# DanMcGann/loam

Measured on AMD Instinct MI355X. Metric: scan-pair registrations/sec (64x1024 Ouster), higher is better.
Workload: dtype f64; 1 GPU; batch of 1024 independent 64x1024 scan pairs per GPU (BASELINE configs[2]/[3]); step = extractFeatures x2 + registerFeatures per pair, inputs resident in HBM; pairs_per_gpu=1024, scan=64x1024, seed=20240311, input_scalar=f64, arithmetic=f64 (float input is widened on load)

## Files before the change

include/loamx.h:

```cpp
#ifndef LOAMX_H_
#define LOAMX_H_

#include <stddef.h>
#include <stdint.h>

#ifdef __cplusplus
extern "C" {
#endif

typedef struct loamx_ctx loamx_ctx;

enum {
  LOAMX_OK = 0,
  LOAMX_ERR_SCAN_SIZE = 1,
  LOAMX_ERR_BAD_PARAM = 2,
  LOAMX_ERR_HIP = 3,
  LOAMX_ERR_CAPACITY = 4,
  LOAMX_ERR_UNSUPPORTED = 5,
  LOAMX_ERR_NO_DEVICE = 6,
  LOAMX_ERR_COMM = 7
};

typedef struct {
  uint64_t scan_lines;
// ... 91 lines not shown
enum {
  LOAMX_WALK_NONE = 0,
  LOAMX_WALK_FLAT = 1,
  LOAMX_WALK_TILED_BY_COUNT = 2,
  LOAMX_WALK_TILED_BY_TILES = 3
};
typedef struct {
  uint32_t iterations, termination;
  uint32_t use_moments;
  uint32_t mom_ref_on;
  double mom_ref[7];
  uint32_t tiles;
  uint32_t live_tiles;
  uint64_t edge_stride, planar_stride;
  uint32_t n_se, n_sp;
  uint32_t walk;
  uint32_t listed_total;
  double s0max, v2max;
  uint32_t sweep_chunk, edge_cache, list_cache, flat_cache;
  uint32_t* tile_counts;
  size_t tile_counts_cap;
} loamx_solve_census;
int loamx_ctx_last_solve_census(loamx_ctx* ctx, size_t pair, loamx_solve_census* out);
enum { LOAMX_ASSOC_SEARCH_NONE = 0, LOAMX_ASSOC_SEARCH_BRUTE = 1, LOAMX_ASSOC_SEARCH_GRID = 2 };
enum { LOAMX_ASSOC_LEFTOVER_NONE = 0, LOAMX_ASSOC_LEFTOVER_LEFT = 1, LOAMX_ASSOC_LEFTOVER_COOP = 2 };
#define LOAMX_ASSOC_REASON_WIDE 0x80000000u
#define LOAMX_ASSOC_REASON_TIED 0x40000000u
typedef struct {
  uint32_t n_src, n_tgt;
  uint64_t stride;
  uint32_t km;
  uint32_t search;
  uint32_t mixed_launch;
  uint32_t one_stage;
  uint32_t leftover_kernel;
  uint32_t rest_blocks, coop_blocks;
  uint32_t rest_spread, left_spread;
  uint32_t lean_set;
  double origin[3], h;
  int32_t nx, ny, nz;
  uint32_t n_points;
  uint32_t verified, unverified, queued_words;
  uint32_t queued, queued_plain, queued_wide, queued_tied;
  uint32_t rest_searched;
  uint32_t listed;
  uint32_t leftover_finished;
// ... 525 lines not shown
```

loam_amd/capi.py:

```python
import collections
import ctypes as C
import os

import numpy as np

from . import build as _build

OK, ERR_SCAN_SIZE, ERR_BAD_PARAM, ERR_HIP, ERR_CAPACITY, ERR_UNSUPPORTED, ERR_NO_DEVICE, ERR_COMM = range(8)
CONVERGED, MAX_ITER, INSUFFICIENT_ASSOCIATIONS = 0, 1, 2
K_CURVATURE, K_SELECT, K_COMPACT, K_GRID, K_ASSOC, K_SWEEP, K_LM, K_MOMENT, K_KNN_PLANE, K_EXTRACT_FUSED, K_INFORMATION, K_CLOUD_ACCUMULATE, K_CLOUD_ACCUMULATE_PLAIN, K_CLOUD_LIST, K_CLOUD_EMIT, K_COUNT = range(16)


class LidarParams(C.Structure):
    _fields_ = [("scan_lines", C.c_uint64), ("points_per_line", C.c_uint64), ("min_range", C.c_double),
                ("max_range", C.c_double)]


class FeatureExtractionParams(C.Structure):
    _fields_ = [("neighbor_points", C.c_uint64), ("number_sectors", C.c_uint64),
                ("max_edge_feats_per_sector", C.c_uint64), ("max_planar_feats_per_sector", C.c_uint64),
                ("edge_feat_threshold", C.c_double), ("planar_feat_threshold", C.c_double),
                ("occlusion_thresh", C.c_double), ("parallel_thresh", C.c_double)]

    def __init__(self, *a, **kw):
# ... 317 lines not shown
PGO_LINEARIZATION_DTYPE = np.dtype([("e", np.float64, 6), ("chi2", np.float64), ("weight", np.float64), ("A", np.float64, (6, 6)),
                                    ("B", np.float64, (6, 6))])
PGO_TERMINATIONS = ("COST_CONVERGED", "STEP_CONVERGED", "MAX_ITERATIONS", "LAMBDA_OVERFLOW", "NOTHING_TO_DO", "BAD_INPUT")
(PGO_COST_CONVERGED, PGO_STEP_CONVERGED, PGO_MAX_ITERATIONS, PGO_LAMBDA_OVERFLOW, PGO_NOTHING_TO_DO, PGO_BAD_INPUT) = range(6)


EXPORTS = [
    "loamx_default_fe_params", "loamx_default_reg_params", "loamx_status_string", "loamx_last_error",
    "loamx_ctx_create", "loamx_ctx_destroy", "loamx_ctx_set_stream", "loamx_ctx_synchronize",
    "loamx_compute_curvature", "loamx_compute_valid_points", "loamx_extract_features", "loamx_register_features",
    "loamx_target_index_create", "loamx_target_index_destroy", "loamx_register_features_indexed",
    "loamx_edge_capacity", "loamx_planar_capacity", "loamx_extract_features_batch_dev",
    "loamx_register_features_batch_dev", "loamx_register_scan_pairs_dev", "loamx_register_scan_pairs",
    "loamx_register_scan_pairs_f32", "loamx_ctx_enable_kernel_timing",
    "loamx_ctx_reset_kernel_stats", "loamx_ctx_get_kernel_stats", "loamx_kernel_name", "loamx_synth_pair_pose",
    "loamx_synth_scan_host", "loamx_synth_scan_pairs_dev", "loamx_dev_alloc", "loamx_dev_free",
    "loamx_copy_to_device", "loamx_copy_to_host",
    "loamx_compute_curvature_f32", "loamx_compute_valid_points_f32", "loamx_extract_features_f32",
    "loamx_extract_features_batch_dev_f32", "loamx_register_scan_pairs_dev_f32",
    "loamx_target_index_insert", "loamx_target_index_size", "loamx_target_index_census",
    "loamx_shard_range", "loamx_comm_get_unique_id", "loamx_comm_create", "loamx_comm_wrap", "loamx_comm_destroy",
    "loamx_comm_info", "loamx_gather_results_dev", "loamx_comm_barrier", "loamx_comm_stats", "loamx_ctx_extract_counters",
    "loamx_ctx_set_option", "loamx_ctx_get_option", "loamx_ctx_last_extract_route", "loamx_ctx_last_solve_census",
    "loamx_ctx_last_assoc_census",
    "loamx_ctx_last_assoc_coop_forms",
    "loamx_fit_lines", "loamx_fit_planes", "loamx_knn_search", "loamx_associate", "loamx_target_index_stats",
    "loamx_register_scan_sequence_dev", "loamx_register_scan_sequence_dev_f32", "loamx_register_scan_sequence",
    "loamx_register_scan_sequence_f32", "loamx_compose_trajectory_dev", "loamx_deskew_scans_dev", "loamx_deskew_scans_dev_f32",
    "loamx_deskew_launch_geometry",
    "loamx_target_index_points", "loamx_voxel_filter_dev", "loamx_target_index_insert_filtered", "loamx_target_index_crop",
    "loamx_registration_information", "loamx_registration_information_indexed", "loamx_registration_information_batch_dev",
    "loamx_register_scan_pairs_info_dev", "loamx_register_scan_pairs_info_dev_f32", "loamx_register_scan_sequence_info_dev",
    "loamx_register_scan_sequence_info_dev_f32",
    "loamx_default_organize_params", "loamx_scan_layout_create", "loamx_scan_layout_destroy", "loamx_scan_layout_tables",
    "loamx_organize_clouds_dev", "loamx_organize_clouds_dev_f32", "loamx_organize_cloud", "loamx_organize_cloud_f32",
    "loamx_default_place_params", "loamx_place_db_create", "loamx_place_db_destroy", "loamx_place_db_sector_dirs", "loamx_place_db_size",
    "loamx_place_descriptors_dev", "loamx_place_descriptors_dev_f32", "loamx_place_db_add_dev", "loamx_place_db_read",
    "loamx_place_search_dev", "loamx_place_descriptor", "loamx_place_descriptor_f32", "loamx_place_search",
    "loamx_pgo_default_params", "loamx_pose_graph_optimize_dev", "loamx_pose_graph_optimize", "loamx_pose_graph_linearize",
    "loamx_pose_graph_edges_from_results_dev",
    "loamx_default_cloud_map_params", "loamx_cloud_map_create", "loamx_cloud_map_destroy", "loamx_cloud_map_clear",
    "loamx_cloud_map_add_clouds_dev", "loamx_cloud_map_add_clouds_dev_f32", "loamx_cloud_map_emit_dev", "loamx_cloud_map_stats_read",
    "loamx_cloud_map_add_cloud", "loamx_cloud_map_add_cloud_f32", "loamx_cloud_map_emit", "loamx_cloud_map_claims_read",
    "loamx_default_segment_params", "loamx_segment_constants", "loamx_segment_scans_dev", "loamx_segment_scans_dev_f32",
    "loamx_segment_scan", "loamx_segment_scan_f32", "loamx_ctx_last_segment_census",
    "loamx_default_visibility_params", "loamx_visibility_votes_dev", "loamx_visibility_votes_dev_f32", "loamx_visibility_filter_dev",
    "loamx_visibility_votes", "loamx_visibility_votes_f32", "loamx_ctx_last_visibility_census",
# ... 177 lines not shown
    lib.loamx_copy_to_host.argtypes = [vp, vp, vp, C.c_size_t]
    szp = C.POINTER(C.c_size_t)
    lib.loamx_shard_range.argtypes = [C.c_size_t, C.c_int, C.c_int, szp, szp]
    lib.loamx_shard_range.restype = None
    lib.loamx_comm_get_unique_id.argtypes = [C.c_char_p]
    lib.loamx_comm_create.argtypes = [vp, C.c_char_p, C.c_int, C.c_int, C.POINTER(vp)]
    lib.loamx_comm_wrap.argtypes = [vp, vp, C.POINTER(vp)]
    lib.loamx_comm_destroy.argtypes = [vp]
    lib.loamx_comm_destroy.restype = None
    lib.loamx_comm_info.argtypes = [vp, C.POINTER(C.c_int), C.POINTER(C.c_int), C.POINTER(C.c_int)]
    lib.loamx_gather_results_dev.argtypes = [vp, vp, vp, C.c_size_t, C.c_size_t, vp]
    lib.loamx_comm_barrier.argtypes = [vp, vp, dp]
    lib.loamx_comm_stats.argtypes = [vp, C.POINTER(C.c_uint64)]
    lib.loamx_ctx_extract_counters.argtypes = [vp, C.POINTER(C.c_uint64), C.POINTER(C.c_uint64)]
    lib.loamx_fit_lines.argtypes = [vp, dp, C.c_size_t, C.c_size_t, dp, dp]
    lib.loamx_fit_planes.argtypes = [vp, dp, C.c_size_t, C.c_size_t, dp, dp]
    lib.loamx_knn_search.argtypes = [vp, vp, C.c_int, dp, C.c_size_t, C.c_size_t, C.c_double, vp, vp]
    lib.loamx_associate.argtypes = [vp, dp, C.c_size_t, dp, C.c_size_t, dp, C.c_size_t, dp, C.c_size_t, dp,
                                    C.POINTER(RegistrationParams), C.POINTER(AssocDump)]
    lib.loamx_ctx_set_option.argtypes = [vp, C.c_char_p, C.c_int]
    lib.loamx_ctx_get_option.argtypes = [vp, C.c_char_p, C.POINTER(C.c_int)]
    lib.loamx_ctx_last_extract_route.argtypes = [vp, C.POINTER(C.c_uint32)]
    lib.loamx_ctx_last_solve_census.argtypes = [vp, C.c_size_t, C.POINTER(SolveCensusStruct)]
    lib.loamx_ctx_last_assoc_census.argtypes = [vp, C.c_int, C.POINTER(AssocCensusStruct)]
    lib.loamx_ctx_last_assoc_coop_forms.argtypes = [vp, C.c_int, u32p]
    lib.loamx_registration_information.argtypes = [vp, dp, C.c_size_t, dp, C.c_size_t, dp, C.c_size_t, dp, C.c_size_t, dp,
                                                   C.POINTER(RegistrationParams), C.POINTER(RegInformation)]
    lib.loamx_registration_information_indexed.argtypes = [vp, vp, dp, C.c_size_t, dp, C.c_size_t, dp, C.POINTER(RegistrationParams),
                                                           C.POINTER(RegInformation)]
    lib.loamx_registration_information_batch_dev.argtypes = lib.loamx_register_features_batch_dev.argtypes
    lib.loamx_register_scan_pairs_info_dev.argtypes = lib.loamx_register_scan_pairs_dev.argtypes + [vp]
    lib.loamx_register_scan_pairs_info_dev_f32.argtypes = lib.loamx_register_scan_pairs_info_dev.argtypes
    lib.loamx_register_scan_sequence_info_dev.argtypes = lib.loamx_register_scan_sequence_dev.argtypes + [vp]
    lib.loamx_register_scan_sequence_info_dev_f32.argtypes = lib.loamx_register_scan_sequence_info_dev.argtypes
    lib.loamx_default_organize_params.argtypes = [C.POINTER(OrganizeParamsStruct)]
    lib.loamx_default_organize_params.restype = None
    lib.loamx_scan_layout_create.argtypes = [vp, C.POINTER(LidarParams), C.POINTER(OrganizeParamsStruct), C.POINTER(vp)]
    lib.loamx_scan_layout_destroy.argtypes = [vp, vp]
    lib.loamx_scan_layout_destroy.restype = None
    lib.loamx_scan_layout_tables.argtypes = [vp, dp, dp]
    lib.loamx_organize_clouds_dev.argtypes = [vp, vp, vp, C.c_size_t, vp, szp, C.c_size_t, vp, vp, vp]
    lib.loamx_organize_clouds_dev_f32.argtypes = lib.loamx_organize_clouds_dev.argtypes
    lib.loamx_organize_cloud.argtypes = [vp, vp, vp, C.c_size_t, vp, C.c_size_t, vp, vp, vp]
    lib.loamx_organize_cloud_f32.argtypes = lib.loamx_organize_cloud.argtypes
    lib.loamx_default_place_params.argtypes = [C.POINTER(PlaceParamsStruct)]
    lib.loamx_default_place_params.restype = None
# ... 591 lines not shown
        self._check(self.lib.loamx_ctx_get_option(self.h, name.encode(), C.byref(v)))
        return v.value

    def extract_counters(self):
        a, b = C.c_uint64(0), C.c_uint64(0)
        self._check(self.lib.loamx_ctx_extract_counters(self.h, C.byref(a), C.byref(b)))
        return a.value, b.value

    def last_extract_route(self):
        v = C.c_uint32(0)
        self._check(self.lib.loamx_ctx_last_extract_route(self.h, C.byref(v)))
        return ExtractRoute(v.value)

    def last_solve_census(self, pair=0):
        v = SolveCensusStruct()
        self._check(self.lib.loamx_ctx_last_solve_census(self.h, pair, C.byref(v)))
        counts = np.zeros(max(1, v.live_tiles), dtype=np.uint32)
        v.tile_counts, v.tile_counts_cap = counts.ctypes.data_as(C.POINTER(C.c_uint32)), v.live_tiles
        self._check(self.lib.loamx_ctx_last_solve_census(self.h, pair, C.byref(v)))
        return SolveCensus(v.iterations, v.termination, v.use_moments, v.mom_ref_on, np.array(list(v.mom_ref)), v.tiles, v.live_tiles,
                           v.edge_stride, v.planar_stride, v.n_se, v.n_sp, v.walk, v.listed_total, v.s0max, v.v2max, v.sweep_chunk,
                           v.edge_cache, v.list_cache, v.flat_cache, counts[:v.live_tiles].copy())

    def last_assoc_coop_forms(self, kind):
        kind = {"edge": 0, "plane": 1}.get(kind, kind)
        out = (C.c_uint32 * 2)()
        self._check(self.lib.loamx_ctx_last_assoc_coop_forms(self.h, kind, out))
        return int(out[0]), int(out[1])

    def last_assoc_census(self, kind):
        kind = {"edge": 0, "plane": 1}.get(kind, kind)
        v = AssocCensusStruct()
        self._check(self.lib.loamx_ctx_last_assoc_census(self.h, kind, C.byref(v)))
        q = int(v.queued)
        eq, er = np.zeros(max(1, q), dtype=np.uint32), np.zeros(max(1, q), dtype=np.uint32)
        ar, bf = np.zeros(max(1, q), dtype=np.int32), np.zeros(max(1, q), dtype=np.int32)
        v.entry_query, v.entry_reason = eq.ctypes.data_as(C.POINTER(C.c_uint32)), er.ctypes.data_as(C.POINTER(C.c_uint32))
        v.count_after_rest, v.count_before_fit = ar.ctypes.data_as(C.POINTER(C.c_int32)), bf.ctypes.data_as(C.POINTER(C.c_int32))
        v.entries_cap = q
        nl = int(v.late)
        lq = np.zeros(max(1, nl), dtype=np.uint32)
        v.late_query, v.late_cap = lq.ctypes.data_as(C.POINTER(C.c_uint32)), nl
        self._check(self.lib.loamx_ctx_last_assoc_census(self.h, kind, C.byref(v)))
        return AssocCensus(*[getattr(v, n) for n in ASSOC_CENSUS_SCALARS], np.array(list(v.origin)), eq[:q].copy(), er[:q].copy(),
                           ar[:q].copy(), bf[:q].copy(), lq[:nl].copy())

# ... 537 lines not shown
```

loam_amd/csrc/api_core.hip:

```cpp
#include "api_host.h"
#include "synth.h"

using namespace loamx;

namespace loamx {
thread_local LaunchScope* g_launch_scope = nullptr;
int g_debug_sync = getenv("LOAMX_DEBUG_SYNC") ? 1 : 0;
thread_local uint32_t g_extract_route = 0;
}

namespace {

const char* kKernelNames[LOAMX_K_COUNT] = {"curvature_valid_kernel", "select_kernel", "compact_kernel",
                                           "grid_build_kernel",      "associate_kernel", "sweep_kernel",
                                           "lm_kernels",             "moment_kernel",    "knn_plane_kernel",
                                           "extract_fused_kernel",   "information_kernel", "cloud_accumulate_kernel",
                                           "cloud_accumulate_plain_kernel", "cloud_list_kernels", "cloud_emit_kernels"};

struct OptionName {
  const char* name;
  bool extract;
  uint32_t bit;
};
const OptionName kOptionNames[] = {
    {"FORCE_TIE_REPLAY", true, kFlagForceReplay}, {"FORCE_SCAN_GIVEUP", true, kFlagForceGiveUp}, {"CURV_V1", true, kFlagCurvV1},
    {"NO_FUSED_COMPACT", true, kFlagNoFusedCompact}, {"NO_MIS_SELECT", true, kFlagNoMisSelect}, {"FUSED_EXTRACT", true, kFlagFusedExtract},
    {"NO_ROW_SELECT", true, kFlagNoRowSelect}, {"FUSED_ROWS", true, kFlagFusedRows}, {"NO_SPLIT_CURV", true, kFlagNoSplitCurv}, {"STAGE_ALWAYS", true, kFlagStageAlways},
    {"NO_MOMENTS", false, kRegFlagNoMoments}, {"NO_PACKED_GRID", false, kRegFlagNoPackedGrid}, {"NO_BIG_GRID", false, kRegFlagNoBigGrid},
    {"NO_GRID_SIDE", false, kRegFlagNoGridSide}, {"DEBUG_POISON", false, kRegFlagPoison},
    {"QUEUE_TWO_STAGE", false, kRegFlagQueueTwoStage}, {"QUEUE_ONE_STAGE", false, kRegFlagQueueOneStage},
    {"NO_MIXED_ASSOC", false, kRegFlagNoMixedAssoc}, {"FORCE_RCCL", false, kRegFlagForceRccl},
    {"NO_COOP_LEFT", false, kRegFlagNoCoopLeft}, {"NO_COOP_ROWS", false, kRegFlagNoCoopRows}, {"NO_REF_MOMENTS", false, kRegFlagNoRefMoments},
    {"NO_EXTRACT_BOXES", false, kRegFlagNoExtractBoxes}, {"CHECK_FINITE", false, kRegFlagCheckFinite},
    {"NO_SMALL_SETS", false, kRegFlagNoSmallSets}, {"FORCE_LATE_VERIFY", false, kRegFlagForceLate},
    {"NO_LIVE_DEAL", false, kRegFlagNoLiveDeal}, {"NO_CLOUDMAP_COMBINE", false, kRegFlagNoCloudmapCombine},
    {"NO_SEGMENT_TILES", false, kRegFlagNoSegmentTiles}, {"NO_VISIBILITY_RANGES", false, kRegFlagNoVisibilityRanges},
    {"NO_OCCUPANCY_COMBINE", false, kRegFlagNoOccupancyCombine}};

}

namespace loamx {

int fail(loamx_ctx* ctx, int code, const std::string& msg) {
  if (ctx) ctx->last_error = msg;
  return code;
}

int ensure(loamx_ctx* ctx, Buf& b, size_t bytes) {
  if (bytes == 0) bytes = 8;
  if (b.cap >= bytes) return LOAMX_OK;
  if (b.p) {
    HIP_TRY(ctx, hipStreamSynchronize(ctx->stream));
    HIP_TRY(ctx, hipFree(b.p));
    b.p = nullptr, b.cap = 0;
  }
  HIP_TRY(ctx, hipMalloc(&b.p, bytes));
  b.cap = bytes;
  return LOAMX_OK;
}
int ensure(loamx_ctx* ctx, int id, size_t bytes) { return ensure(ctx, ctx->ws[id], bytes); }
// ... 424 lines not shown
```

loam_amd/csrc/api_register.hip:

```cpp
#include "api_host.h"

using namespace loamx;

namespace {

int enqueue_association(loamx_ctx* ctx, const RegBatch& B, const RegConfig& C, uint32_t what = kAssocEdges | kAssocPlanes,
                        AssocCensusRun* census = nullptr) {
  hipStream_t s = ctx->stream;
  {
    TimedScope t(ctx, LOAMX_K_ASSOC, 0.0);
    const bool side = (size_t)B.n_pairs * B.kind[kPlane].assoc_blocks >= 128;
    PendingEvent knn{};
    LaunchScope knn_ls{nullptr, nullptr, true};
    if (ctx->timing) {
      knn.kernel = LOAMX_K_KNN_PLANE, knn.bytes = 0.0, knn.own_e0 = true;
      knn.e0 = take_event(ctx), knn.e1 = take_event(ctx);
      knn_ls = LaunchScope{knn.e0, knn.e1, true};
    }
    launch_associate(B, C, s, side ? ctx->aux_stream : nullptr, side ? ctx->aux2_stream : nullptr, ctx->ev_fork, ctx->ev_mid, ctx->ev_join,
                     ctx->ev_join2, ctx->timing ? &knn_ls : nullptr, what, census);
    if (ctx->timing) {
      if (knn_ls.first) ctx->event_pool.push_back(knn.e0), ctx->event_pool.push_back(knn.e1);
      else ctx->pending.push_back(knn);
    }
// ... 11 lines not shown
#ifdef LOAMX_NN_SAME_STATS
  debug_nn_same(B, it, s);
#endif
  if (hook) {
    untimed(ctx);
    int rc = hook(ctx, B, it, hook_user);
    if (rc != LOAMX_OK) return rc;
  }
  {
    TimedScope t(ctx, LOAMX_K_LM, 0.0, true);
    launch_lm_begin(B, C, s);
  }
  const bool ref_first = it == 0 && B.ref_moments != 0u;
  if (ref_first) {
    {
      TimedScope t(ctx, LOAMX_K_SWEEP, 0.0, true);
      launch_sweep(B, s);
    }
    TimedScope t(ctx, LOAMX_K_LM, 0.0, true);
    launch_lm_step(B, s);
  }
  if (it > 0 || ref_first) {
    TimedScope t(ctx, LOAMX_K_MOMENT, 0.0, true);
    launch_moments(B, s);
  }
  if (it > 0 || ref_first) {
    TimedScope t(ctx, LOAMX_K_LM, 0.0, true);
    launch_lm_pair_loop(B, C, s);
  } else {
    for (int k = 0; k < 5; k++) {
      {
        TimedScope t(ctx, LOAMX_K_SWEEP, 0.0, true);
        launch_sweep(B, s);
      }
      {
        TimedScope t(ctx, LOAMX_K_LM, 0.0, true);
        launch_lm_step(B, s);
      }
    }
  }
  CHECK_LAUNCH(ctx, "sweep/lm kernels");
  if (it == 0 && !ref_first) {
    TimedScope t(ctx, LOAMX_K_LM, 0.0, true);
    launch_outer_update(B, C, s);
  }
  CHECK_LAUNCH(ctx, "outer_update_kernel");
  return LOAMX_OK;
// ... 456 lines not shown
  out->tiles = B.mom_blocks_per_pair * 4;
  out->edge_stride = B.kind[kEdge].stride, out->planar_stride = B.kind[kPlane].stride;
  out->n_se = n_raw[kEdge] < B.kind[kEdge].stride ? n_raw[kEdge] : (uint32_t)B.kind[kEdge].stride;
  out->n_sp = n_raw[kPlane] < B.kind[kPlane].stride ? n_raw[kPlane] : (uint32_t)B.kind[kPlane].stride;
  out->sweep_chunk = (uint32_t)kSweepChunk, out->edge_cache = kEdgeCache, out->list_cache = kListCache, out->flat_cache = kFlatCache;
  uint32_t live = 0;
  while (live < out->tiles && (size_t)(live / 4) * kSweepChunk < out->n_sp) live++;
  out->live_tiles = live;
  const bool lists = !(ctx->last_solve_flags & kRegFlagNoMoments) && (S.iterations >= 2u || S.mom_ref_on != 0u);
  if (!lists) return LOAMX_OK;
  double maxima[2];
  HIP_TRY(ctx, hipMemcpy(maxima, B.moments + pair * (size_t)(kMomSize + 2) + kMomSize, sizeof(maxima), hipMemcpyDeviceToHost));
  out->s0max = maxima[0], out->v2max = maxima[1];
  std::vector<uint32_t> cnt(live);
  if (live) HIP_TRY(ctx, hipMemcpy(cnt.data(), B.flagged_count + pair * (size_t)out->tiles, live * sizeof(uint32_t), hipMemcpyDeviceToHost));
  for (uint32_t t = 0; t < live; t++) {
    out->listed_total += cnt[t];
    if (t < cap) counts_out[t] = cnt[t];
  }
  out->walk = out->tiles > kListCache ? LOAMX_WALK_TILED_BY_TILES : (out->listed_total > kFlatCache ? LOAMX_WALK_TILED_BY_COUNT : LOAMX_WALK_FLAT);
  return LOAMX_OK;
}

int loamx_ctx_last_assoc_census(loamx_ctx* ctx, int which_kind, loamx_assoc_census* out) {
  if (!out) return LOAMX_ERR_BAD_PARAM;
  API_LOCK(ctx);
  if (which_kind != 0 && which_kind != 1) return fail(ctx, LOAMX_ERR_BAD_PARAM, "which_kind: 0 = edges, 1 = planes");
  if (!ctx->last_assoc_census_valid) return fail(ctx, LOAMX_ERR_BAD_PARAM, "no association dump on this context to read (or another call came after it)");
  const loamx_ctx::AssocCensusKept& keep = ctx->last_assoc_census[which_kind];
  uint32_t *const eq = out->entry_query, *const er = out->entry_reason;
  int32_t *const ar = out->count_after_rest, *const bf = out->count_before_fit;
  const size_t cap = out->entries_cap, lcap = out->late_cap;
  uint32_t* const lq = out->late_query;
  *out = keep.c;
  out->late_query = lq, out->late_cap = lcap;
  for (size_t t = 0; lq && t < keep.late.size() && t < lcap; t++) lq[t] = keep.late[t];
  out->entry_query = eq, out->entry_reason = er, out->count_after_rest = ar, out->count_before_fit = bf, out->entries_cap = cap;
  for (size_t t = 0; t < keep.entry.size() && t < cap; t++) {
    if (eq) eq[t] = keep.entry[t] & 0x3FFFFFFFu;
    if (er) er[t] = keep.entry[t] & (LOAMX_ASSOC_REASON_WIDE | LOAMX_ASSOC_REASON_TIED);
    if (ar) ar[t] = keep.after_rest[t];
    if (bf) bf[t] = keep.before_fit[t];
  }
  return LOAMX_OK;
}

// ... 146 lines not shown
```

loam_amd/csrc/loamx_internal.h:

```cpp
#pragma once
#include <hip/hip_runtime.h>
#include <hip/hip_ext.h>
#include <stdint.h>
#include <stdio.h>

#include <vector>

#include "../../include/loamx.h"
#include "extract_math.h"
#include "reg_math.h"
#include "organize_math.h"
#include "place_math.h"
#include "segment_math.h"
#include "visibility_math.h"
#include "occupancy_math.h"
#include "xcd_map.h"

namespace loamx {

struct LaunchScope {
  hipEvent_t start, stop;
  bool first;
};
extern thread_local LaunchScope* g_launch_scope;
// ... 85 lines not shown
  RegKindConfig kind[2];
  double min_line_cond, max_avg_plane_dist;
  uint32_t max_iterations;
  double rot_thresh, pos_thresh;
  uint32_t min_associations;
  uint32_t flags;
};
constexpr uint32_t kRegFlagNoMoments = 1u;
constexpr uint32_t kRegFlagNoPackedGrid = 2u;
constexpr uint32_t kRegFlagNoBigGrid = 4u;
constexpr uint32_t kRegFlagNoGridSide = 8u;
constexpr uint32_t kRegFlagPoison = 16u;
constexpr uint32_t kRegFlagQueueTwoStage = 32u;
constexpr uint32_t kRegFlagQueueOneStage = 64u;
constexpr uint32_t kRegFlagForceRccl = 256u;
constexpr uint32_t kRegFlagNoCoopLeft = 512u;
constexpr uint32_t kRegFlagNoCoopRows = 131072u;
constexpr uint32_t kRegFlagNoRefMoments = 1024u;
constexpr uint32_t kRegFlagNoSmallSets = 8192u;
constexpr uint32_t kRegFlagCheckFinite = 4096u;
constexpr uint32_t kRegFlagNoExtractBoxes = 2048u;
constexpr uint32_t kRegFlagNoMixedAssoc = 128u;
constexpr uint32_t kRegFlagNoLiveDeal = 32768u;
constexpr uint32_t kRegFlagForceLate = 16384u;

struct GridSet {
  GridDesc* desc;
  uint32_t* cell_start;
  GridPoint* sorted;
  size_t stride;
  float* rel;
  uint32_t cells_cap;
};

struct RegKind {
  size_t stride;
  const double* src;
  const uint32_t* n_src;
  const double* tgt;
  const uint32_t* n_tgt;
  GridSet grid;
  GridSet src_grid;
  uint32_t knn_mode;
  uint32_t assoc_blocks;
  double* rec;
  uint32_t* nn;
// ... 95 lines not shown
};
struct AssocCensusBuf {
  uint32_t* counts;
  int32_t* after_rest;
  int32_t* before_fit;
};
struct AssocCensusRun {
  AssocCensusForm form[2];
  AssocCensusBuf buf[2];
};
void assoc_census_derive(const AssocCensusForm& F, size_t n_pairs, const GridDesc& g, const uint32_t* rest, uint32_t queued, uint32_t listed,
                         uint32_t out[4]);
constexpr uint32_t kAssocEdges = 1u, kAssocPlanes = 2u;
void launch_associate(const RegBatch& B, const RegConfig& C, hipStream_t s, hipStream_t aux, hipStream_t aux2, hipEvent_t ev_fork,
                      hipEvent_t ev_mid, hipEvent_t ev_join, hipEvent_t ev_join2, LaunchScope* knn_scope = nullptr,
                      uint32_t what = kAssocEdges | kAssocPlanes, AssocCensusRun* census = nullptr);
#ifdef LOAMX_NN_SAME_STATS
void debug_nn_same(const RegBatch& B, uint32_t it, hipStream_t s);
#endif
void launch_lm_begin(const RegBatch& B, const RegConfig& C, hipStream_t s);
void launch_sweep(const RegBatch& B, hipStream_t s);
void launch_lm_pair_loop(const RegBatch& B, const RegConfig& C, hipStream_t s);
void launch_lm_step(const RegBatch& B, hipStream_t s);
void launch_moments(const RegBatch& B, hipStream_t s);
void launch_outer_update(const RegBatch& B, const RegConfig& C, hipStream_t s);
void launch_write_results(const RegBatch& B, loamx_reg_result* d_results, hipStream_t s);

size_t index_insert_ws_bytes(size_t cells, size_t n_add);
void launch_index_insert_count(const GridSet& gs, size_t cells, const double* d_add, uint32_t n_add, void* ws, hipStream_t s);
void launch_index_insert_merge(const GridSet& gs, size_t cells, uint32_t n_old, const double* d_add, uint32_t n_add, void* ws,
                               GridPoint* sorted2, float* rel2, hipStream_t s);

constexpr int kFitMaxK = 32;
struct AssocDumpSet {
  uint32_t* nn_count;
  uint32_t* nn_idx;
  uint8_t* valid;
  double* moved;
  double* prim;
};
void launch_fit_sets(bool plane, const double* d_pts, size_t n_sets, int k, double* d_prim, double* d_aux, hipStream_t s);
void launch_knn_queries(const GridSet& gs, const double* d_q, size_t n_q, int k, double max_dist, uint32_t* d_idx, uint32_t* d_count,
                        hipStream_t s);
void launch_assoc_dump(const RegBatch& B, const RegConfig& C, const AssocDumpSet (&out)[2], hipStream_t s);

struct InfoPartial {
  double s[28];
// ... 209 lines not shown
```

loam_amd/csrc/reg_math.h:

```cpp
#pragma once
#include <stdint.h>

#if defined(__HIPCC__)
#include <hip/hip_runtime.h>
#include <math.h>
#define LOAMX_HD __host__ __device__ __forceinline__
#else
#include <math.h>
#define LOAMX_HD inline
#endif

namespace loamx {

constexpr int kMaxK = 16;
constexpr double kDblMin = 2.2250738585072014e-308;
constexpr double kDblMax = 1.7976931348623157e308;
constexpr double kDblEps = 2.220446049250313e-16;

struct Vec3 {
  double x, y, z;
};
LOAMX_HD Vec3 v3(double x, double y, double z) { return Vec3{x, y, z}; }
LOAMX_HD Vec3 vadd(Vec3 a, Vec3 b) { return Vec3{a.x + b.x, a.y + b.y, a.z + b.z}; }
LOAMX_HD Vec3 vsub(Vec3 a, Vec3 b) { return Vec3{a.x - b.x, a.y - b.y, a.z - b.z}; }
// ... 2170 lines not shown
#pragma unroll
  for (int i = 0; i < 6; i++) {
#pragma unroll
    for (int j = i; j < 6; j++) acc[t++] += J[i] * J[j];
  }
#pragma unroll
  for (int j = 0; j < 6; j++) acc[21 + j] += J[j] * f;
  acc[27] += 0.5 * rho0;
}

constexpr int kMomDim = 13;
constexpr int kMomStride = 16;
constexpr int kMomSize = kMomStride * kMomStride;
constexpr double kMomInlier = 0.5;
LOAMX_HD void plane_coeffs(Vec3 v, Vec3 n, double d, double c[kMomDim]) {
  const double nv = vdot(n, v);
  c[0] = nv - d;
  const Vec3 m = vcross(v, n);
  c[1] = m.x, c[2] = m.y, c[3] = m.z;
  c[4] = 2.0 * n.x * v.x - 2.0 * nv, c[5] = 2.0 * n.y * v.y - 2.0 * nv, c[6] = 2.0 * n.z * v.z - 2.0 * nv;
  c[7] = 2.0 * (n.x * v.y + n.y * v.x), c[8] = 2.0 * (n.x * v.z + n.z * v.x), c[9] = 2.0 * (n.y * v.z + n.z * v.y);
  c[10] = n.x, c[11] = n.y, c[12] = n.z;
}
LOAMX_HD void plane_eval_from_moments(const double* M, const double x[7], double acc[29]) {
  const double ux = x[0], uy = x[1], uz = x[2], w = x[3];
  double phi[kMomDim] = {1.0, 2.0 * w * ux, 2.0 * w * uy, 2.0 * w * uz, ux * ux, uy * uy, uz * uz,
                         ux * uy, ux * uz, uy * uz, x[4], x[5], x[6]};
  double A[kMomDim][4];
#pragma unroll
  for (int j = 0; j < kMomDim; j++) A[j][0] = A[j][1] = A[j][2] = A[j][3] = 0.0;
  A[1][0] = 2.0 * w, A[1][3] = 2.0 * ux;
  A[2][1] = 2.0 * w, A[2][3] = 2.0 * uy;
  A[3][2] = 2.0 * w, A[3][3] = 2.0 * uz;
  A[4][0] = 2.0 * ux, A[5][1] = 2.0 * uy, A[6][2] = 2.0 * uz;
  A[7][0] = uy, A[7][1] = ux;
  A[8][0] = uz, A[8][2] = ux;
  A[9][1] = uz, A[9][2] = uy;
  const double W = x[0], X = x[1], Y = x[2], Zq = x[3];
  double Z[kMomDim][6];
#pragma unroll
  for (int j = 0; j < kMomDim; j++) {
    Z[j][0] = A[j][0] * (-X) + A[j][1] * W + A[j][2] * (-Zq) + A[j][3] * Y;
    Z[j][1] = A[j][0] * (-Y) + A[j][1] * Zq + A[j][2] * W + A[j][3] * (-X);
    Z[j][2] = A[j][0] * (-Zq) + A[j][1] * (-Y) + A[j][2] * X + A[j][3] * W;
    Z[j][3] = j == 10 ? 1.0 : 0.0, Z[j][4] = j == 11 ? 1.0 : 0.0, Z[j][5] = j == 12 ? 1.0 : 0.0;
  }
// ... 300 lines not shown
```

loam_amd/csrc/register_kernels.hip:

```cpp
#include "loamx_internal.h"

namespace loamx {

namespace {

__device__ __forceinline__ double wave_min(double v) {
#pragma unroll
  for (int off = 32; off >= 1; off >>= 1) v = fmin(v, __shfl_xor(v, off));
  return v;
}
__device__ __forceinline__ double wave_max(double v) {
#pragma unroll
  for (int off = 32; off >= 1; off >>= 1) v = fmax(v, __shfl_xor(v, off));
  return v;
}

#ifndef LOAMX_BUILD_THREADS
#define LOAMX_BUILD_THREADS 1024
#endif
constexpr int kBuildThreads = LOAMX_BUILD_THREADS;

template <bool ORDERED, bool PACKED>
__global__ __launch_bounds__(kBuildThreads) void grid_build_kernel(const double* __restrict__ pts_base,
                                                                   const uint32_t* __restrict__ n_pts, size_t stride,
// ... 1786 lines not shown
  {
    double xr[7];
#pragma unroll
    for (int i = 0; i < 7; i++) xr[i] = ref_on ? S.mom_ref[i] : (i == 3 ? 1.0 : 0.0);
    plane_phi(xr, phi_ref);
  }
  uint32_t* __restrict__ flist = B.flagged_list + ((pair * B.mom_blocks_per_pair + blk) * 4 + wave) * (size_t)(kSweepChunk / 4);
  uint32_t n_flagged = 0;
  struct Rec {
    double f[7];
    bool in;
  };
  auto load_rec = [&](uint32_t q) {
    Rec R;
    R.in = q < n_sp;
#pragma unroll
    for (int f = 0; f < 7; f++) R.f[f] = R.in ? Pl[f * pfield + q] : 0.0;
    return R;
  };
  constexpr int kIters = kSweepChunk / kSweepThreads;
  Rec cur = load_rec(base + tix);
#pragma unroll 1
  for (int it = 0; it < kIters; it++) {
    const Rec nxt = (it + 1 < kIters) ? load_rec(base + (it + 1) * kSweepThreads + tix) : Rec{{0, 0, 0, 0, 0, 0, 0}, false};
    double c[kMomDim];
#pragma unroll
    for (int j = 0; j < kMomDim; j++) c[j] = 0.0;
    bool flagged = false;
    if (cur.in && cur.f[0] == cur.f[0]) {
      const Vec3 v = v3(cur.f[0], cur.f[1], cur.f[2]);
      plane_coeffs(v, v3(cur.f[3], cur.f[4], cur.f[5]), cur.f[6], c);
      double sref = c[0];
      if (ref_on) {
        sref = 0.0;
#pragma unroll
        for (int j = 0; j < kMomDim; j++) sref += c[j] * phi_ref[j];
      }
      const double a0 = fabs(sref), vv = vdot(v, v);
      flagged = !(a0 <= kMomInlier);
      if (flagged) {
#pragma unroll
        for (int j = 0; j < kMomDim; j++) c[j] = 0.0;
      } else {
        s0max = a0 > s0max ? a0 : s0max;
        v2max = vv > v2max ? vv : v2max;
      }
    }
    const unsigned long long fm = __ballot(flagged);
    if (flagged) flist[n_flagged + (uint32_t)__popcll(fm & ((1ull << lane) - 1ull))] = base + it * kSweepThreads + tix;
    n_flagged += (uint32_t)__popcll(fm);
    __builtin_amdgcn_fence(__ATOMIC_RELEASE, "wavefront");
    __builtin_amdgcn_wave_barrier();
#pragma unroll
    for (int j = 0; j < kMomDim; j++) tile[j][lane] = c[j];
    __builtin_amdgcn_fence(__ATOMIC_RELEASE, "wavefront");
    __builtin_amdgcn_wave_barrier();
    __builtin_amdgcn_fence(__ATOMIC_ACQUIRE, "wavefront");
#pragma unroll
    for (int t = 0; t < 16; t++) {
      const double a = tile[lane & 15][4 * t + (lane >> 4)];
      acc = __builtin_amdgcn_mfma_f64_16x16x4f64(a, a, acc, 0, 0, 0);
    }
    cur = nxt;
  }
  double* __restrict__ out = B.mom_partials + ((pair * B.mom_blocks_per_pair + blk) * 4 + wave) * (size_t)(kMomSize + 2);
#pragma unroll
  for (int r = 0; r < 4; r++) out[((lane >> 4) + 4 * r) * kMomStride + (lane & 15)] = acc[r];
  s0max = wave_max(s0max), v2max = wave_max(v2max);
  if (lane == 0) out[kMomSize] = s0max, out[kMomSize + 1] = v2max;
  if (lane == 0) B.flagged_count[(pair * B.mom_blocks_per_pair + blk) * 4 + wave] = n_flagged;
}

__global__ void outer_update_kernel(RegBatch B, RegConfig C) {
  const size_t pair = (size_t)blockIdx.x * blockDim.x + threadIdx.x;
  if (pair >= B.n_pairs) return;
  PairState& S = B.state[pair];
  if (!S.active) return;
  outer_update_pair(B, C, pair, S);
}

__global__ void write_results_kernel(RegBatch B, loamx_reg_result* __restrict__ out) {
  const size_t pair = (size_t)blockIdx.x * blockDim.x + threadIdx.x;
  if (pair >= B.n_pairs) return;
  if (pair == 0 && B.max_counts) {
    for (int c = 0; c < 4; c++) B.max_counts[c] = 0u;
    B.max_counts[4] = B.max_counts[5] = 0xFFFFFFFFu;
  }
  const PairState& S = B.state[pair];
  for (int i = 0; i < 7; i++) out[pair].pose[i] = S.est[i];
  out[pair].termination = S.termination;
// ... 448 lines not shown
  static unsigned long long* stats = nullptr;
  const size_t words = 6 * B.n_pairs * B.kind[kPlane].stride;
  if (!prev) { (void)hipMalloc(&prev, words * 4); (void)hipMalloc(&stats, 24); }
  (void)hipMemsetAsync(stats, 0, 24, s);
  launch_kernel(nn_same_kernel, dim3((unsigned)((B.kind[kPlane].stride + 255) / 256), (unsigned)B.n_pairs), dim3(256), 0, s, B, prev, stats, it);
  unsigned long long h[3];
  (void)hipMemcpyAsync(h, stats, 24, hipMemcpyDeviceToHost, s);
  (void)hipStreamSynchronize(s);
  printf("nn_same it=%u: %llu active plane queries, %llu keep their list (%.1f %%), %llu queued (%.1f %%)\n", it, h[0], h[1],
         100.0 * (double)h[1] / (double)(h[0] ? h[0] : 1), h[2], 100.0 * (double)h[2] / (double)(h[0] ? h[0] : 1));
}
#endif

void launch_sweep(const RegBatch& B, hipStream_t s) {
  if (B.n_pairs == 0 || B.blocks_per_pair == 0) return;
  launch_kernel(sweep_kernel, dim3((unsigned)(B.n_pairs * B.blocks_per_pair)), dim3(kSweepThreads), 0, s, B);
}

void launch_lm_pair_loop(const RegBatch& B, const RegConfig& C, hipStream_t s) {
  if (B.n_pairs == 0) return;
  launch_kernel(lm_pair_loop_kernel, dim3((unsigned)B.n_pairs), dim3(64), 0, s, B, C);
}

void launch_moments(const RegBatch& B, hipStream_t s) {
  if (B.n_pairs == 0 || B.mom_blocks_per_pair == 0) return;
  launch_kernel(moment_kernel, dim3((unsigned)(B.n_pairs * B.mom_blocks_per_pair * 4)), dim3(64), 0, s, B);
}

void launch_lm_step(const RegBatch& B, hipStream_t s) {
  if (B.n_pairs == 0) return;
  launch_kernel(lm_step_kernel, dim3(per_pair_grid(B.n_pairs)), dim3(64), 0, s, B);
}

void launch_lm_begin(const RegBatch& B, const RegConfig& C, hipStream_t s) {
  if (B.n_pairs == 0) return;
  launch_kernel(lm_begin_kernel, dim3(per_pair_grid(B.n_pairs)), dim3(64), 0, s, B, C);
}

void launch_outer_update(const RegBatch& B, const RegConfig& C, hipStream_t s) {
  if (B.n_pairs == 0) return;
  launch_kernel(outer_update_kernel, dim3(per_pair_grid(B.n_pairs)), dim3(64), 0, s, B, C);
}

void launch_write_results(const RegBatch& B, loamx_reg_result* d_results, hipStream_t s) {
  if (B.n_pairs == 0) return;
  launch_kernel(write_results_kernel, dim3(per_pair_grid(B.n_pairs)), dim3(64), 0, s, B, d_results);
}

}
// ... 1 lines not shown
```

Baseline: 109,200 pairs/s.

## Accumulate plane moments per lane with FMAs instead of MFMA outer products

Adds a moment kernel where each lane accumulates the upper triangle of its own 13x13 moment outer product with scalar FMAs. Row 0 is kept in LDS to limit register pressure, and a sliced LDS reduction with shuffles builds the symmetric tile at the end. This replaces the per-iteration LDS transpose plus f64 MFMA. The new kernel becomes the default, the MFMA path stays behind an option flag, and both kernels now exit early for empty chunks. The large per-lane accumulator array risks register spills and lower occupancy. A debug API to read the final moments is also added.

```diff
diff --git a/include/loamx.h b/include/loamx.h
--- a/include/loamx.h
+++ b/include/loamx.h
@@ -137,6 +137,7 @@
   size_t tile_counts_cap;
 } loamx_solve_census;
 int loamx_ctx_last_solve_census(loamx_ctx* ctx, size_t pair, loamx_solve_census* out);
+int loamx_ctx_last_solve_moments(loamx_ctx* ctx, size_t pair, double out[258]);
 enum { LOAMX_ASSOC_SEARCH_NONE = 0, LOAMX_ASSOC_SEARCH_BRUTE = 1, LOAMX_ASSOC_SEARCH_GRID = 2 };
 enum { LOAMX_ASSOC_LEFTOVER_NONE = 0, LOAMX_ASSOC_LEFTOVER_LEFT = 1, LOAMX_ASSOC_LEFTOVER_COOP = 2 };
 #define LOAMX_ASSOC_REASON_WIDE 0x80000000u
diff --git a/loam_amd/capi.py b/loam_amd/capi.py
--- a/loam_amd/capi.py
+++ b/loam_amd/capi.py
@@ -363,7 +363,7 @@
     "loamx_shard_range", "loamx_comm_get_unique_id", "loamx_comm_create", "loamx_comm_wrap", "loamx_comm_destroy",
     "loamx_comm_info", "loamx_gather_results_dev", "loamx_comm_barrier", "loamx_comm_stats", "loamx_ctx_extract_counters",
     "loamx_ctx_set_option", "loamx_ctx_get_option", "loamx_ctx_last_extract_route", "loamx_ctx_last_solve_census",
-    "loamx_ctx_last_assoc_census",
+    "loamx_ctx_last_solve_moments", "loamx_ctx_last_assoc_census",
     "loamx_ctx_last_assoc_coop_forms",
     "loamx_fit_lines", "loamx_fit_planes", "loamx_knn_search", "loamx_associate", "loamx_target_index_stats",
     "loamx_register_scan_sequence_dev", "loamx_register_scan_sequence_dev_f32", "loamx_register_scan_sequence",
@@ -587,6 +587,7 @@
     lib.loamx_ctx_get_option.argtypes = [vp, C.c_char_p, C.POINTER(C.c_int)]
     lib.loamx_ctx_last_extract_route.argtypes = [vp, C.POINTER(C.c_uint32)]
     lib.loamx_ctx_last_solve_census.argtypes = [vp, C.c_size_t, C.POINTER(SolveCensusStruct)]
+    lib.loamx_ctx_last_solve_moments.argtypes = [vp, C.c_size_t, dp]
     lib.loamx_ctx_last_assoc_census.argtypes = [vp, C.c_int, C.POINTER(AssocCensusStruct)]
     lib.loamx_ctx_last_assoc_coop_forms.argtypes = [vp, C.c_int, u32p]
     lib.loamx_registration_information.argtypes = [vp, dp, C.c_size_t, dp, C.c_size_t, dp, C.c_size_t, dp, C.c_size_t, dp,
@@ -1224,6 +1225,11 @@
                            v.edge_stride, v.planar_stride, v.n_se, v.n_sp, v.walk, v.listed_total, v.s0max, v.v2max, v.sweep_chunk,
                            v.edge_cache, v.list_cache, v.flat_cache, counts[:v.live_tiles].copy())
 
+    def last_solve_moments(self, pair=0):
+        out = np.zeros(258, dtype=np.float64)
+        self._check(self.lib.loamx_ctx_last_solve_moments(self.h, pair, out.ctypes.data_as(C.POINTER(C.c_double))))
+        return out[:256].reshape(16, 16).copy(), float(out[256]), float(out[257])
+
     def last_assoc_coop_forms(self, kind):
         kind = {"edge": 0, "plane": 1}.get(kind, kind)
         out = (C.c_uint32 * 2)()
diff --git a/loam_amd/csrc/api_core.hip b/loam_amd/csrc/api_core.hip
--- a/loam_amd/csrc/api_core.hip
+++ b/loam_amd/csrc/api_core.hip
@@ -35,7 +35,7 @@
     {"NO_SMALL_SETS", false, kRegFlagNoSmallSets}, {"FORCE_LATE_VERIFY", false, kRegFlagForceLate},
     {"NO_LIVE_DEAL", false, kRegFlagNoLiveDeal}, {"NO_CLOUDMAP_COMBINE", false, kRegFlagNoCloudmapCombine},
     {"NO_SEGMENT_TILES", false, kRegFlagNoSegmentTiles}, {"NO_VISIBILITY_RANGES", false, kRegFlagNoVisibilityRanges},
-    {"NO_OCCUPANCY_COMBINE", false, kRegFlagNoOccupancyCombine}};
+    {"NO_OCCUPANCY_COMBINE", false, kRegFlagNoOccupancyCombine}, {"MFMA_MOMENTS", false, kRegFlagMfmaMoments}};
 
 }
 
diff --git a/loam_amd/csrc/api_register.hip b/loam_amd/csrc/api_register.hip
--- a/loam_amd/csrc/api_register.hip
+++ b/loam_amd/csrc/api_register.hip
@@ -57,7 +57,7 @@
   }
   if (it > 0 || ref_first) {
     TimedScope t(ctx, LOAMX_K_MOMENT, 0.0, true);
-    launch_moments(B, s);
+    launch_moments(B, C, s);
   }
   if (it > 0 || ref_first) {
     TimedScope t(ctx, LOAMX_K_LM, 0.0, true);
@@ -560,6 +560,18 @@
   return LOAMX_OK;
 }
 
+int loamx_ctx_last_solve_moments(loamx_ctx* ctx, size_t pair, double out[258]) {
+  if (!out) return LOAMX_ERR_BAD_PARAM;
+  loamx_solve_census cen{};
+  const int rc = loamx_ctx_last_solve_census(ctx, pair, &cen);
+  if (rc != LOAMX_OK) return rc;
+  API_ENTER(ctx);
+  if (cen.walk == LOAMX_WALK_NONE) return fail(ctx, LOAMX_ERR_BAD_PARAM, "no moment pass ran for this pair in its last iteration");
+  static_assert(kMomSize + 2 == 258, "loamx.h states the size");
+  HIP_TRY(ctx, hipMemcpy(out, ctx->last_solve_batch.moments + pair * (size_t)(kMomSize + 2), (kMomSize + 2) * sizeof(double), hipMemcpyDeviceToHost));
+  return LOAMX_OK;
+}
+
 int loamx_ctx_last_assoc_census(loamx_ctx* ctx, int which_kind, loamx_assoc_census* out) {
   if (!out) return LOAMX_ERR_BAD_PARAM;
   API_LOCK(ctx);
diff --git a/loam_amd/csrc/loamx_internal.h b/loam_amd/csrc/loamx_internal.h
--- a/loam_amd/csrc/loamx_internal.h
+++ b/loam_amd/csrc/loamx_internal.h
@@ -131,6 +131,7 @@
 constexpr uint32_t kRegFlagNoExtractBoxes = 2048u;
 constexpr uint32_t kRegFlagNoMixedAssoc = 128u;
 constexpr uint32_t kRegFlagNoLiveDeal = 32768u;
+constexpr uint32_t kRegFlagMfmaMoments = 2097152u;
 constexpr uint32_t kRegFlagForceLate = 16384u;
 
 struct GridSet {
@@ -272,7 +273,7 @@
 void launch_sweep(const RegBatch& B, hipStream_t s);
 void launch_lm_pair_loop(const RegBatch& B, const RegConfig& C, hipStream_t s);
 void launch_lm_step(const RegBatch& B, hipStream_t s);
-void launch_moments(const RegBatch& B, hipStream_t s);
+void launch_moments(const RegBatch& B, const RegConfig& C, hipStream_t s);
 void launch_outer_update(const RegBatch& B, const RegConfig& C, hipStream_t s);
 void launch_write_results(const RegBatch& B, loamx_reg_result* d_results, hipStream_t s);
 
diff --git a/loam_amd/csrc/reg_math.h b/loam_amd/csrc/reg_math.h
--- a/loam_amd/csrc/reg_math.h
+++ b/loam_amd/csrc/reg_math.h
@@ -2216,6 +2216,68 @@
   c[7] = 2.0 * (n.x * v.y + n.y * v.x), c[8] = 2.0 * (n.x * v.z + n.z * v.x), c[9] = 2.0 * (n.y * v.z + n.z * v.y);
   c[10] = n.x, c[11] = n.y, c[12] = n.z;
 }
+
+constexpr int kMomTri = kMomDim * (kMomDim + 1) / 2;
+constexpr int kMomSlice = 16;
+constexpr int kMomSlices = (kMomTri + kMomSlice - 1) / kMomSlice;
+LOAMX_HD bool moment_record(const double f[7], bool in, bool ref_on, const double phi_ref[kMomDim], double c[kMomDim], double& s0max,
+                            double& v2max) {
+  const bool there = in && f[0] == f[0];
+  const Vec3 v = v3(f[0], f[1], f[2]);
+  plane_coeffs(v, v3(f[3], f[4], f[5]), f[6], c);
+  double sref = c[0];
+  if (ref_on) {
+    sref = 0.0;
+#pragma unroll
+    for (int j = 0; j < kMomDim; j++) sref += c[j] * phi_ref[j];
+  }
+  const double a0 = fabs(sref), vv = vdot(v, v);
+  const bool keep = there && a0 <= kMomInlier;
+#pragma unroll
+  for (int j = 0; j < kMomDim; j++) c[j] = keep ? c[j] : 0.0;
+  s0max = keep && a0 > s0max ? a0 : s0max;
+  v2max = keep && vv > v2max ? vv : v2max;
+  return there && !keep;
+}
+template <int R0, int R1>
+LOAMX_HD void moment_lane_add_rows(const double c[kMomDim], double* acc) {
+  int e = 0;
+#pragma unroll
+  for (int i = R0; i < R1; i++) {
+#pragma unroll
+    for (int j = i; j < kMomDim; j++, e++) acc[e] = __builtin_fma(c[i], c[j], acc[e]);
+  }
+}
+LOAMX_HD void moment_lane_add(const double c[kMomDim], double acc[kMomTri]) { moment_lane_add_rows<0, kMomDim>(c, acc); }
+LOAMX_HD void moment_tri_index(int e, int& i, int& j) {
+  i = 0;
+  while (e >= kMomDim - i) e -= kMomDim - i, i++;
+  j = i + e;
+}
+LOAMX_HD double moment_quarter_sum(const double* x) {
+  double p = x[0];
+#pragma unroll
+  for (int m = 1; m < 16; m++) p += x[m];
+  return p;
+}
+template <int NQ>
+LOAMX_HD double moment_join_quarters(const double (&p)[NQ]) {
+#if defined(__HIP_DEVICE_COMPILE__)
+  static_assert(NQ == 1, "a device lane holds its own quarter");
+  const double t = p[0] + __shfl_xor(p[0], 1);
+  return t + __shfl_xor(t, 2);
+#else
+  if constexpr (NQ == 4) return (p[0] + p[1]) + (p[2] + p[3]);
+  else return p[0];
+#endif
+}
+LOAMX_HD void moment_tile_put(double* tile, int e, double v) {
+  int i, j;
+  moment_tri_index(e, i, j);
+  tile[i * kMomStride + j] = v, tile[j * kMomStride + i] = v;
+}
+LOAMX_HD bool moment_tile_padding(int idx) { return idx / kMomStride >= kMomDim || idx % kMomStride >= kMomDim; }
+
 LOAMX_HD void plane_eval_from_moments(const double* M, const double x[7], double acc[29]) {
   const double ux = x[0], uy = x[1], uz = x[2], w = x[3];
   double phi[kMomDim] = {1.0, 2.0 * w * ux, 2.0 * w * uy, 2.0 * w * uz, ux * ux, uy * uy, uz * uz,
diff --git a/loam_amd/csrc/register_kernels.hip b/loam_amd/csrc/register_kernels.hip
--- a/loam_amd/csrc/register_kernels.hip
+++ b/loam_amd/csrc/register_kernels.hip
@@ -1832,6 +1832,7 @@
   Rec cur = load_rec(base + tix);
 #pragma unroll 1
   for (int it = 0; it < kIters; it++) {
+    if (base + (uint32_t)(it * kSweepThreads + wave * 64) >= n_sp) break;
     const Rec nxt = (it + 1 < kIters) ? load_rec(base + (it + 1) * kSweepThreads + tix) : Rec{{0, 0, 0, 0, 0, 0, 0}, false};
     double c[kMomDim];
 #pragma unroll
@@ -1876,6 +1877,121 @@
   double* __restrict__ out = B.mom_partials + ((pair * B.mom_blocks_per_pair + blk) * 4 + wave) * (size_t)(kMomSize + 2);
 #pragma unroll
   for (int r = 0; r < 4; r++) out[((lane >> 4) + 4 * r) * kMomStride + (lane & 15)] = acc[r];
+  s0max = wave_max(s0max), v2max = wave_max(v2max);
+  if (lane == 0) out[kMomSize] = s0max, out[kMomSize + 1] = v2max;
+  if (lane == 0) B.flagged_count[(pair * B.mom_blocks_per_pair + blk) * 4 + wave] = n_flagged;
+}
+
+__device__ __forceinline__ double uniform_f64(double v) {
+  const long long b = __double_as_longlong(v);
+  return __longlong_as_double(((long long)__builtin_amdgcn_readfirstlane((int)(b >> 32)) << 32) |
+                              (unsigned int)__builtin_amdgcn_readfirstlane((int)(b & 0xFFFFFFFFll)));
+}
+
+__global__ __launch_bounds__(64, 2) void moment_lanes_kernel(RegBatch B) {
+  __shared__ double s_red[kMomSlice][kMomLdsRow];
+  __shared__ double s_row0[kMomDim][64];
+  const int wave = (int)(blockIdx.x & 3u), lane = (int)threadIdx.x;
+  const int tix = wave * 64 + lane;
+  size_t pair = (blockIdx.x >> 2) / B.mom_blocks_per_pair;
+  const uint32_t blk = (blockIdx.x >> 2) % B.mom_blocks_per_pair;
+  {
+    uint32_t n_live;
+    const uint32_t* live = live_list(B, 1u, n_live);
+    if (live) {
+      if (pair >= n_live) return;
+      pair = live[pair];
+      if (pair >= B.n_pairs) return;
+    }
+  }
+  const PairState& S = B.state[pair];
+  if (!S.active || !S.lm.active || !S.use_moments) return;
+  const uint32_t n_sp_raw = B.kind[kPlane].n_src[pair * B.in_pitch];
+  const uint32_t n_sp = n_sp_raw < B.kind[kPlane].stride ? n_sp_raw : (uint32_t)B.kind[kPlane].stride;
+  const uint32_t base = blk * kSweepChunk;
+  if (base >= n_sp) return;
+  if (blk == 0 && tix == 0 && B.sweep_slots) atomicAdd(&B.sweep_slots[4], (unsigned long long)n_sp);
+  const size_t pfield = B.n_pairs * B.kind[kPlane].stride;
+  const double* __restrict__ Pl = B.kind[kPlane].rec + pair * B.kind[kPlane].stride;
+  const bool ref_on = S.mom_ref_on != 0u;
+  double phi_ref[kMomDim];
+  {
+    double xr[7];
+#pragma unroll
+    for (int i = 0; i < 7; i++) xr[i] = ref_on ? S.mom_ref[i] : (i == 3 ? 1.0 : 0.0);
+    plane_phi(xr, phi_ref);
+#pragma unroll
+    for (int j = 0; j < kMomDim; j++) phi_ref[j] = uniform_f64(phi_ref[j]);
+  }
+  uint32_t* __restrict__ flist = B.flagged_list + ((pair * B.mom_blocks_per_pair + blk) * 4 + wave) * (size_t)(kSweepChunk / 4);
+  uint32_t n_flagged = 0;
+  double s0max = 0.0, v2max = 0.0;
+  double acc[kMomTri - kMomDim];
+#pragma unroll
+  for (int e = 0; e < kMomTri - kMomDim; e++) acc[e] = 0.0;
+#pragma unroll
+  for (int j = 0; j < kMomDim; j++) s_row0[j][lane] = 0.0;
+  struct Rec {
+    double f[7];
+  };
+  const uint32_t lim = n_sp < base + kSweepChunk ? n_sp : base + kSweepChunk;
+  auto load_rec = [&](uint32_t q) {
+    Rec R;
+    const uint32_t qc = q < lim ? q : lim - 1u;
+#pragma unroll
+    for (int f = 0; f < 7; f++) R.f[f] = Pl[f * pfield + qc];
+    return R;
+  };
+  constexpr int kIters = kSweepChunk / kSweepThreads;
+  const uint32_t first = base + (uint32_t)tix;
+  Rec cur = load_rec(first);
+  Rec nxt = load_rec(first + (uint32_t)kSweepThreads);
+#pragma unroll 1
+  for (int it = 0; it < kIters; it++) {
+    const uint32_t group = base + (uint32_t)(it * kSweepThreads + wave * 64);
+    if (group >= n_sp) break;
+    const Rec nx2 = load_rec(first + (uint32_t)((it + 2) * kSweepThreads));
+    double c[kMomDim];
+    const bool flagged = moment_record(cur.f, first + (uint32_t)(it * kSweepThreads) < n_sp, ref_on, phi_ref, c, s0max, v2max);
+    const unsigned long long fm = __ballot(flagged);
+    if (flagged) flist[n_flagged + (uint32_t)__popcll(fm & ((1ull << lane) - 1ull))] = base + it * kSweepThreads + tix;
+    n_flagged += (uint32_t)__popcll(fm);
+    {
+      double row0[kMomDim];
+#pragma unroll
+      for (int j = 0; j < kMomDim; j++) row0[j] = s_row0[j][lane];
+      moment_lane_add_rows<0, 1>(c, row0);
+#pragma unroll
+      for (int j = 0; j < kMomDim; j++) s_row0[j][lane] = row0[j];
+    }
+    moment_lane_add_rows<1, kMomDim>(c, acc);
+    cur = nxt, nxt = nx2;
+  }
+  double row0[kMomDim];
+#pragma unroll
+  for (int j = 0; j < kMomDim; j++) row0[j] = s_row0[j][lane];
+  double* __restrict__ out = B.mom_partials + ((pair * B.mom_blocks_per_pair + blk) * 4 + wave) * (size_t)(kMomSize + 2);
+#pragma unroll
+  for (int r = 0; r < kMomSize / 64; r++)
+    if (moment_tile_padding(lane + 64 * r)) out[lane + 64 * r] = 0.0;
+#pragma unroll
+  for (int sl = 0; sl < kMomSlices; sl++) {
+    __builtin_amdgcn_fence(__ATOMIC_RELEASE, "wavefront");
+    __builtin_amdgcn_wave_barrier();
+#pragma unroll
+    for (int k = 0; k < kMomSlice; k++) {
+      const int e = sl * kMomSlice + k;
+      if (e < kMomDim) s_red[k][lane] = row0[e];
+      else if (e < kMomTri) s_red[k][lane] = acc[e - kMomDim];
+    }
+    __builtin_amdgcn_fence(__ATOMIC_RELEASE, "wavefront");
+    __builtin_amdgcn_wave_barrier();
+    __builtin_amdgcn_fence(__ATOMIC_ACQUIRE, "wavefront");
+    const int e = sl * kMomSlice + (lane >> 2);
+    const double quarter[1] = {e < kMomTri ? moment_quarter_sum(&s_red[lane >> 2][16 * (lane & 3)]) : 0.0};
+    const double v = moment_join_quarters(quarter);
+    if ((lane & 3) == 0 && e < kMomTri) moment_tile_put(out, e, v);
+  }
   s0max = wave_max(s0max), v2max = wave_max(v2max);
   if (lane == 0) out[kMomSize] = s0max, out[kMomSize + 1] = v2max;
   if (lane == 0) B.flagged_count[(pair * B.mom_blocks_per_pair + blk) * 4 + wave] = n_flagged;
@@ -2370,9 +2486,11 @@
   launch_kernel(lm_pair_loop_kernel, dim3((unsigned)B.n_pairs), dim3(64), 0, s, B, C);
 }
 
-void launch_moments(const RegBatch& B, hipStream_t s) {
+void launch_moments(const RegBatch& B, const RegConfig& C, hipStream_t s) {
   if (B.n_pairs == 0 || B.mom_blocks_per_pair == 0) return;
-  launch_kernel(moment_kernel, dim3((unsigned)(B.n_pairs * B.mom_blocks_per_pair * 4)), dim3(64), 0, s, B);
+  const dim3 grid((unsigned)(B.n_pairs * B.mom_blocks_per_pair * 4));
+  if (C.flags & kRegFlagMfmaMoments) launch_kernel(moment_kernel, grid, dim3(64), 0, s, B);
+  else launch_kernel(moment_lanes_kernel, grid, dim3(64), 0, s, B);
 }
 
 void launch_lm_step(const RegBatch& B, hipStream_t s) {
```

After: 109,200 pairs/s. Within noise of the previous version (-0.0%).
